# thangvubk/SoftGroup

Measured on AMD Instinct MI355X. Metric: scans/sec ScanNet-v2-like inference (softgroup_scannet.yaml, full forward_test), higher is better.
Workload: dtype f32

## Files before the change

### softgroup_amd/csrc/ballquery.hip

```cpp
#include "common.h"
#include "scan.h"

namespace sg {

constexpr int32_t kBqEmpty = 0x7f7f7f7f;
constexpr int kBqBuf = 2048;
constexpr int kBqCap = SG_BALLQUERY_MAX_NEIGHBORS;
constexpr int kBqKeep = 64;

struct BqWs {
  int4 *cell;
  int32_t *table;
  int32_t *count;
  int32_t *start;
  int32_t *cursor;
  int32_t *slot_of;
  float4 *sorted;
  int32_t *keep;
  void *scan_ws;
  size_t scan_bytes;
  uint32_t cap;
};

__device__ __forceinline__ uint32_t cell_slot(int b, int cx, int cy, int cz, uint32_t mask) {
  uint64_t h = (static_cast<uint64_t>(static_cast<uint32_t>(b)) << 32) | static_cast<uint32_t>(cx);
  h = mix64(h) ^ ((static_cast<uint64_t>(static_cast<uint32_t>(cy)) << 32) | static_cast<uint32_t>(cz));
  return static_cast<uint32_t>(mix64(h)) & mask;
}

__global__ void __launch_bounds__(256) bq_insert_kernel(const float *__restrict__ xyz,
                                                       const int32_t *__restrict__ batch_idxs,
                                                       int n, double inv_cell, int4 *__restrict__ cell,
                                                       int32_t *table, uint32_t mask, int32_t *count,
                                                       int32_t *__restrict__ slot_of) {
  const int i = blockIdx.x * 256 + threadIdx.x;
  if (i >= n) return;
  int4 c;
  c.x = batch_idxs ? batch_idxs[i] : 0;
  c.y = static_cast<int>(floor(static_cast<double>(xyz[3 * i + 0]) * inv_cell));
  c.z = static_cast<int>(floor(static_cast<double>(xyz[3 * i + 1]) * inv_cell));
  c.w = static_cast<int>(floor(static_cast<double>(xyz[3 * i + 2]) * inv_cell));
  cell[i] = c;
  uint32_t s = cell_slot(c.x, c.y, c.z, c.w, mask);
  while (true) {
    int32_t cur = __hip_atomic_load(&table[s], __ATOMIC_RELAXED, __HIP_MEMORY_SCOPE_AGENT);
    if (cur == kBqEmpty) {
      cur = atomicCAS(&table[s], kBqEmpty, i);
      if (cur == kBqEmpty) break;
    }
    int4 o;
    o.x = batch_idxs ? batch_idxs[cur] : 0;
    o.y = static_cast<int>(floor(static_cast<double>(xyz[3 * cur + 0]) * inv_cell));
    o.z = static_cast<int>(floor(static_cast<double>(xyz[3 * cur + 1]) * inv_cell));
    o.w = static_cast<int>(floor(static_cast<double>(xyz[3 * cur + 2]) * inv_cell));
    if (o.x == c.x && o.y == c.y && o.z == c.z && o.w == c.w) break;
    s = (s + 1) & mask;
  }
  slot_of[i] = static_cast<int32_t>(s);
  atomicAdd(&count[s], 1);
}

__global__ void __launch_bounds__(256) bq_scatter_kernel(const float *__restrict__ xyz, int n,
                                                        const int32_t *__restrict__ slot_of,
                                                        const int32_t *__restrict__ start,
                                                        int32_t *cursor, float4 *__restrict__ sorted) {
  const int i = blockIdx.x * 256 + threadIdx.x;
  if (i >= n) return;
  const int s = slot_of[i];
  const int pos = start[s] + atomicAdd(&cursor[s], 1);
  sorted[pos] = make_float4(xyz[3 * i], xyz[3 * i + 1], xyz[3 * i + 2], __int_as_float(i));
}

__device__ __forceinline__ float dist2(float ox, float oy, float oz, float x, float y, float z) {
  const float dx = __fsub_rn(ox, x), dy = __fsub_rn(oy, y), dz = __fsub_rn(oz, z);
  return __fmaf_rn(dz, dz, __fmaf_rn(dx, dx, __fmul_rn(dy, dy)));
}

struct BqCells {
  int start, excl, incl, total;
};
__device__ __forceinline__ BqCells bq_cells(int my_start, int my_count) {
  BqCells c;
  c.start = my_start;
  c.incl = wave_incl_scan(my_count);
  c.excl = c.incl - my_count;
  c.total = __shfl(c.incl, 63, 64);
  return c;
}
__device__ __forceinline__ int bq_candidate(const BqCells &c, int t) {
  int lo = 0, hi = 26;
#pragma unroll
  for (int it = 0; it < 5; ++it) {
    const int mid = (lo + hi) >> 1;
    const bool right = __shfl(c.incl, mid, 64) <= t;
    lo = right ? mid + 1 : lo;
    hi = right ? hi : mid;
  }
  return __shfl(c.start, lo, 64) + (t - __shfl(c.excl, lo, 64));
}

__device__ __forceinline__ int bq_scan_count(const float4 *__restrict__ sorted, const BqCells &c,
                                             float ox, float oy, float oz, float r2, int limit) {
  int total = 0;
  for (int t0 = 0; t0 < c.total; t0 += 64) {
    const int t = t0 + lane_id();
    const int at = bq_candidate(c, min(t, c.total - 1));
    if (t < c.total) {
      const float4 p = sorted[at];
      total += (dist2(ox, oy, oz, p.x, p.y, p.z) < r2 && __float_as_int(p.w) < limit) ? 1 : 0;
    }
  }
  return wave_sum(total);
}

template <bool FILL>
__global__ void __launch_bounds__(256) bq_query_kernel(const float *__restrict__ xyz, int n,
                                                      float r2, const int4 *__restrict__ cell,
                                                      const int32_t *__restrict__ table,
                                                      const int32_t *__restrict__ count,
                                                      const int32_t *__restrict__ start,
                                                      uint32_t mask, const float4 *__restrict__ sorted,
                                                      int32_t *__restrict__ start_len,
                                                      int32_t *__restrict__ idx_out, int32_t *__restrict__ keep) {
  __shared__ __attribute__((aligned(16))) int32_t buf_all[FILL ? 4 * kBqBuf : 4 * kBqKeep];
  const int wave = threadIdx.x >> 6, lane = threadIdx.x & 63;
  int32_t *buf = buf_all + wave * (FILL ? kBqBuf : kBqKeep);
  for (int i = blockIdx.x * 4 + wave; i < n; i += gridDim.x * 4) {
    if (FILL) {
      const int out_len = start_len[2 * i + 1];
      if (out_len <= kBqKeep) {
        if (lane < out_len) idx_out[static_cast<int64_t>(start_len[2 * i]) + lane] = keep[static_cast<int64_t>(i) * kBqKeep + lane];
        continue;
      }
    }
    const float ox = xyz[3 * i], oy = xyz[3 * i + 1], oz = xyz[3 * i + 2];
    const int4 c = cell[i];
    int my_start = 0, my_count = 0;
    if (lane < 27) {
      const int cx = c.y + lane / 9 - 1, cy = c.z + (lane / 3) % 3 - 1, cz = c.w + lane % 3 - 1;
      uint32_t s = cell_slot(c.x, cx, cy, cz, mask);
      while (true) {
        const int32_t rep = table[s];
        if (rep == kBqEmpty) break;
        const int4 o = cell[rep];
        if (o.x == c.x && o.y == cx && o.z == cy && o.w == cz) {
          my_start = start[s];
          my_count = count[s];
          break;
        }
        s = (s + 1) & mask;
      }
    }
    const BqCells cells = bq_cells(my_start, my_count);
    if (!FILL) {
      int m = 0;
      for (int t0 = 0; t0 < cells.total; t0 += 64) {
        const int t = t0 + lane;
        const int at = bq_candidate(cells, min(t, cells.total - 1));
        bool ok = false;
        int id = 0;
        if (t < cells.total) {
          const float4 p = sorted[at];
          id = __float_as_int(p.w);
          ok = dist2(ox, oy, oz, p.x, p.y, p.z) < r2;
        }
        const uint64_t bal = __ballot(ok);
        const int pos = m + mask_prefix(bal);
        if (ok && pos < kBqKeep) buf[pos] = id;
        m += __popcll(bal);
      }
      if (lane == 0) start_len[2 * i + 1] = min(m, kBqCap);
      if (m <= kBqKeep) {
        __builtin_amdgcn_fence(__ATOMIC_RELEASE, "wavefront");
        __builtin_amdgcn_wave_barrier();
        const int e = lane < m ? buf[lane] : 0x7fffffff;
        int rank = 0;
        for (int j = 0; j < m; ++j) rank += (buf[j] < e);
        if (lane < m) keep[static_cast<int64_t>(i) * kBqKeep + rank] = e;
      }
      __builtin_amdgcn_wave_barrier();
      continue;
    }
    const int out_start = start_len[2 * i], out_len = start_len[2 * i + 1];
    int limit = 0x7fffffff;
    int m = 0;
    for (int attempt = 0; attempt < 2; ++attempt) {
      m = 0;
      for (int t0 = 0; t0 < cells.total; t0 += 64) {
        const int t = t0 + lane;
        const int at = bq_candidate(cells, min(t, cells.total - 1));
        bool ok = false;
        int id = 0;
        if (t < cells.total) {
          const float4 p = sorted[at];
          id = __float_as_int(p.w);
          ok = dist2(ox, oy, oz, p.x, p.y, p.z) < r2 && id < limit;
        }
        const uint64_t bal = __ballot(ok);
        const int pos = m + mask_prefix(bal);
        if (ok && pos < kBqBuf) buf[pos] = id;
        m += __popcll(bal);
      }
      if (m <= kBqBuf) break;
      int lo = 0, hi = n;
      while (lo < hi) {
        const int mid = lo + (hi - lo) / 2;
        const int cmid = bq_scan_count(sorted, cells, ox, oy, oz, r2, mid);
        if (cmid >= out_len) hi = mid; else lo = mid + 1;
      }
      limit = lo;
    }
    __builtin_amdgcn_fence(__ATOMIC_RELEASE, "wavefront");
    __builtin_amdgcn_wave_barrier();
    for (int e0 = 0; e0 < m; e0 += 64) {
      const int ei = e0 + lane;
      const int e = ei < m ? buf[ei] : 0x7fffffff;
      int rank = 0;
      int j = 0;
      for (; j + 4 <= m; j += 4) {
        const int4 q = *reinterpret_cast<const int4 *>(buf + j);
        rank += (q.x < e) + (q.y < e) + (q.z < e) + (q.w < e);
      }
      for (; j < m; ++j) rank += (buf[j] < e);
      if (ei < m && rank < out_len) idx_out[static_cast<int64_t>(out_start) + rank] = e;
    }
    __builtin_amdgcn_wave_barrier();
  }
}

static size_t bq_cap(int n) {
  size_t cap = 1024;
  while (cap < static_cast<size_t>(n) * 2) cap <<= 1;
  return cap;
}

static bool bq_carve(void *ws, size_t ws_bytes, int n, BqWs *w) {
  Workspace a(ws, ws_bytes);
  const size_t nn = static_cast<size_t>(n > 0 ? n : 1);
  w->cap = static_cast<uint32_t>(bq_cap(n));
  w->cell = a.take<int4>(nn);
  w->sorted = a.take<float4>(nn);
  w->table = a.take<int32_t>(w->cap);
  w->count = a.take<int32_t>(w->cap);
  w->start = a.take<int32_t>(w->cap);
  w->cursor = a.take<int32_t>(w->cap);
  w->slot_of = a.take<int32_t>(nn);
  w->scan_bytes = scan_workspace_bytes(w->cap);
  w->scan_ws = a.take<char>(w->scan_bytes);
  w->keep = a.take<int32_t>(nn * kBqKeep);
  return w->scan_ws != nullptr && w->keep != nullptr;
}

}

using namespace sg;

extern "C" {

size_t sg_ballquery_workspace_bytes(int n) {
  const size_t nn = static_cast<size_t>(n > 0 ? n : 1);
  const size_t cap = bq_cap(n);
  return 2 * align_up(nn * 16) + 4 * align_up(cap * 4) + align_up(nn * 4) +
         align_up(scan_workspace_bytes(cap)) + align_up(nn * kBqKeep * 4) + 256;
}

int sg_ballquery_build_grid(const float *xyz, const int32_t *batch_idxs, int n, float radius,
                            void *ws, size_t ws_bytes, sg_stream_t stream_) {
  SG_REQUIRE(n >= 0 && radius > 0.f, "sg_ballquery_build_grid: bad arguments (n=%d r=%g)", n, radius);
  hipStream_t stream = as_stream(stream_);
  BqWs w;
  if (!bq_carve(ws, ws_bytes, n, &w)) {
    set_error("sg_ballquery_build_grid: workspace too small");
    return SG_ERR_WORKSPACE;
  }
  if (n == 0) return SG_OK;
  {
    FillList f;
    f.add(w.table, static_cast<size_t>(w.cap) * 4, 0x7f);
    f.add(w.count, static_cast<size_t>(w.cap) * 4, 0);
    f.add(w.cursor, static_cast<size_t>(w.cap) * 4, 0);
    fill_many(f, stream);
  }
  const double inv_cell = 1.0 / (static_cast<double>(radius) * (1.0 + 1e-6));
  const int grid = (n + 255) / 256;
  bq_insert_kernel<<<grid, 256, 0, stream>>>(xyz, batch_idxs, n, inv_cell, w.cell, w.table,
                                             w.cap - 1, w.count, w.slot_of);
  const int32_t *count = w.count;
  int32_t *start = w.start;
  auto in = [count] __device__(int64_t s) { return count[s]; };
  auto out = [start] __device__(int64_t s, int v) { start[s] = v; };
  int rc = exclusive_scan(in, out, w.cap, nullptr, w.scan_ws, w.scan_bytes, stream);
  if (rc != SG_OK) return rc;
  bq_scatter_kernel<<<grid, 256, 0, stream>>>(xyz, n, w.slot_of, w.start, w.cursor, w.sorted);
  return check_launch("sg_ballquery_build_grid");
}

int sg_ballquery_count(const float *xyz, const int32_t *batch_idxs, int n, float radius,
                       int32_t *start_len, int32_t *meta, void *ws, size_t ws_bytes,
                       sg_stream_t stream_) {
  (void)batch_idxs;
  (void)meta;
  SG_REQUIRE(n >= 0 && radius > 0.f, "sg_ballquery_count: bad arguments");
  BqWs w;
  if (!bq_carve(ws, ws_bytes, n, &w)) {
    set_error("sg_ballquery_count: workspace too small");
    return SG_ERR_WORKSPACE;
  }
  if (n == 0) return SG_OK;
  const float r2 = radius * radius;
  bq_query_kernel<false><<<grid_for(n, 4, 256 * 16), 256, 0, as_stream(stream_)>>>(
      xyz, n, r2, w.cell, w.table, w.count, w.start, w.cap - 1, w.sorted, start_len, nullptr, w.keep);
  return check_launch("sg_ballquery_count");
}

int sg_ballquery_fill(const float *xyz, const int32_t *batch_idxs, int n, float radius,
                      const int32_t *start_len, int32_t *idx, void *ws, size_t ws_bytes,
                      sg_stream_t stream_) {
  (void)batch_idxs;
  SG_REQUIRE(n >= 0 && radius > 0.f, "sg_ballquery_fill: bad arguments");
  BqWs w;
  if (!bq_carve(ws, ws_bytes, n, &w)) {
    set_error("sg_ballquery_fill: workspace too small");
    return SG_ERR_WORKSPACE;
  }
  if (n == 0) return SG_OK;
  const float r2 = radius * radius;
  bq_query_kernel<true><<<grid_for(n, 4, 256 * 16), 256, 0, as_stream(stream_)>>>(
      xyz, n, r2, w.cell, w.table, w.count, w.start, w.cap - 1, w.sorted,
      const_cast<int32_t *>(start_len), idx, w.keep);
  return check_launch("sg_ballquery_fill");
}

}
```

### softgroup_amd/csrc/bfs.hip

```cpp
#include <stdlib.h>

#include <map>
#include <mutex>
#include <utility>

#include "common.h"
#include "scan.h"

namespace sg {

constexpr int kCap = SG_BALLQUERY_MAX_NEIGHBORS;
constexpr int kEmitThreads = 512;
constexpr int kEmitWaves = kEmitThreads / 64;

#define SG_LD(p) __hip_atomic_load((p), __ATOMIC_RELAXED, __HIP_MEMORY_SCOPE_AGENT)
#define SG_ST(p, v) __hip_atomic_store((p), (v), __ATOMIC_RELAXED, __HIP_MEMORY_SCOPE_AGENT)

struct BfsWs {
  int32_t *parent, *lab, *size, *cid, *coff, *owner, *seeds, *ebase, *wcnt, *asym_nodes;
  int4 *label;
  int2 *erec;
  int32_t *counters;
  void *scan_ws;
  size_t scan_bytes;
// ... 1 lines not shown
  unsigned long long *big_rec[2];
};

constexpr int kBigFastWgs = 16;
constexpr int kBigSlice = 8192;
constexpr int kBigClusterMin = 16384;
inline bool big_fast_on() {
  const char *e = getenv("SG_BFS_BIG_FAST");
  return !(e && atoi(e) == 0);
}
inline int thin_levels_on() {
  const char *e = getenv("SG_BFS_THIN");
  return e ? atoi(e) : 0;
}
inline bool big_local_on() {
  const char *e = getenv("SG_BFS_BIG_LOCAL");
  return !(e && atoi(e) == 0);
}
inline size_t big_stage_entries(int n) {
  return n > kBigClusterMin && big_fast_on() ? static_cast<size_t>(n) + static_cast<size_t>(kBigFastWgs) * kBigSlice : 0;
}

static bool bfs_carve(void *ws, size_t ws_bytes, int n, int64_t n_edges, BfsWs *w) {
  Workspace a(ws, ws_bytes);
  const size_t nn = static_cast<size_t>(n > 0 ? n : 1);
  w->parent = a.take<int32_t>(nn);
  w->lab = a.take<int32_t>(nn);
  w->label = a.take<int4>(nn);
  w->size = a.take<int32_t>(nn);
  w->cid = a.take<int32_t>(nn);
  w->coff = a.take<int32_t>(nn);
  w->owner = a.take<int32_t>(nn);
  w->seeds = a.take<int32_t>(nn);
  w->ebase = a.take<int32_t>(nn);
  w->wcnt = a.take<int32_t>(nn);
  w->asym_nodes = a.take<int32_t>(nn);
  w->counters = a.take<int32_t>(64);
  w->scan_bytes = scan_workspace_bytes(n);
  w->scan_ws = a.take<char>(w->scan_bytes);
  w->erec = a.take<int2>(static_cast<size_t>(n_edges > 0 ? n_edges : 1));
  bool ok = w->scan_ws != nullptr && w->erec != nullptr;
  const size_t be = big_stage_entries(n);
  for (int i = 0; i < 2; ++i) {
    w->big_stage[i] = be ? a.take<int32_t>(be) : nullptr;
    w->big_rec[i] = be ? a.take<unsigned long long>(be) : nullptr;
    ok = ok && (be == 0 || (w->big_stage[i] != nullptr && w->big_rec[i] != nullptr));
  }
  return ok;
}

__device__ __forceinline__ int uf_find(int32_t *parent, int x) {
  int cur = SG_LD(&parent[x]);
  if (cur != x) {
    int prev = x, next;
    while (cur > (next = SG_LD(&parent[cur]))) {
      SG_ST(&parent[prev], next);
      prev = cur;
      cur = next;
    }
  }
  return cur;
}

__device__ __forceinline__ void uf_union(int32_t *parent, int a, int b) {
  while (a != b) {
    if (a < b) { const int t = a; a = b; b = t; }
    const int old = atomicCAS(&parent[a], a, b);
    if (old == a) return;
    a = uf_find(parent, old);
    b = uf_find(parent, b);
  }
}

__device__ __forceinline__ bool list_has_sorted(const int32_t *__restrict__ lst, int len, int key) {
  int lo = 0, hi = len;
  while (lo < hi) {
    const int mid = (lo + hi) >> 1;
    const int v = lst[mid];
    if (v < key) lo = mid + 1; else hi = mid;
  }
  return lo < len && lst[lo] == key;
}

__global__ void __launch_bounds__(256) bfs_init_kernel(int n, int32_t *parent, int32_t *size,
                                                      int32_t *owner) {
  const int i = blockIdx.x * 256 + threadIdx.x;
  if (i < n) {
    parent[i] = i;
    size[i] = 0;
    owner[i] = 0x7fffffff;
  }
}

constexpr int kSample = 2;
template <int SAMPLE>
__global__ void __launch_bounds__(256) bfs_union_kernel(const int32_t *__restrict__ idx,
                                                       const int32_t *__restrict__ start_len, int n,
                                                       int lists_sorted, int radius_lists,
                                                       int32_t *parent, int32_t *asym_nodes,
                                                       int32_t *counters) {
  const int wave = threadIdx.x >> 6, lane = threadIdx.x & 63;
  for (int u = blockIdx.x * 4 + wave; u < n; u += gridDim.x * 4) {
    const int st = start_len[2 * u], ln_all = start_len[2 * u + 1];
    const int ln = SAMPLE ? min(ln_all, kSample) : ln_all;
    const bool u_capped = ln_all >= kCap;
    bool any_asym = false;
    const int ru = SAMPLE ? -1 : SG_LD(&parent[u]);
    for (int p0 = 0; p0 < ln; p0 += 64) {
      const int p = p0 + lane;
      const int v = p < ln ? idx[st + p] : u;
      bool sym = true;
      if (v != u) {
        const int vst = start_len[2 * v], vln = start_len[2 * v + 1];
        if (!radius_lists || u_capped || vln >= kCap) {
          if (lists_sorted) {
            sym = list_has_sorted(idx + vst, vln, u);
          } else {
            sym = false;
            for (int j = 0; j < vln; ++j)
              if (idx[vst + j] == u) { sym = true; break; }
          }
        }
        if (sym) {
          if (v < u && (SAMPLE || SG_LD(&parent[v]) != ru)) uf_union(parent, uf_find(parent, u), uf_find(parent, v));
        }
      }
      any_asym |= !sym;
    }
    if (!SAMPLE && __any(any_asym)) {
      if (lane == 0) asym_nodes[atomicAdd(&counters[0], 1)] = u;
    }
  }
}

__global__ void __launch_bounds__(256) bfs_hook_min_kernel(const int32_t *__restrict__ idx,
                                                          const int32_t *__restrict__ start_len, int n,
                                                          int lists_sorted, int radius_lists, int32_t *parent) {
  const int u = blockIdx.x * 256 + threadIdx.x;
  if (u >= n) return;
  const int st = start_len[2 * u], ln = start_len[2 * u + 1];
  if (ln == 0 || !lists_sorted) return;
  const int v = idx[st];
  if (v >= u) return;
  if (!radius_lists || ln >= kCap || start_len[2 * v + 1] >= kCap)
    if (!list_has_sorted(idx + start_len[2 * v], start_len[2 * v + 1], u)) return;
  parent[u] = v;
}
__global__ void __launch_bounds__(256) bfs_compress_kernel(int n, int32_t *parent) {
  const int i = blockIdx.x * 256 + threadIdx.x;
  if (i < n) SG_ST(&parent[i], uf_find(parent, i));
}

__global__ void __launch_bounds__(256) bfs_flatten_kernel(int n, int32_t *parent, int32_t *lab) {
  const int i = blockIdx.x * 256 + threadIdx.x;
  if (i >= n) return;
  int r = i;
  while (true) {
    const int p = SG_LD(&parent[r]);
    if (p == r) break;
    r = p;
  }
  lab[i] = r;
}
__global__ void __launch_bounds__(256) bfs_store_root_kernel(int n, const int32_t *__restrict__ lab,
                                                            int32_t *__restrict__ parent) {
  const int i = blockIdx.x * 256 + threadIdx.x;
  if (i < n) parent[i] = lab[i];
}

__global__ void __launch_bounds__(256) bfs_propagate_kernel(const int32_t *__restrict__ idx,
                                                           const int32_t *__restrict__ start_len,
                                                           const int32_t *__restrict__ asym_nodes,
                                                           int n_asym,
                                                           const int32_t *__restrict__ root_of,
                                                           int32_t *lab, int32_t *counters) {
  const int wave = threadIdx.x >> 6, lane = threadIdx.x & 63;
  for (int a = blockIdx.x * 4 + wave; a < n_asym; a += gridDim.x * 4) {
    const int u = asym_nodes[a];
    const int ru = root_of[u];
    const int st = start_len[2 * u], ln = start_len[2 * u + 1];
    for (int p = lane; p < ln; p += 64) {
      const int rv = root_of[idx[st + p]];
      if (rv == ru) continue;
      const int lu = SG_LD(&lab[ru]);
      if (lu < SG_LD(&lab[rv])) {
        if (atomicMin(&lab[rv], lu) > lu) SG_ST(&counters[1], 1);
      }
    }
  }
}

__global__ void __launch_bounds__(256) bfs_label_kernel(int n, const int32_t *__restrict__ root_of,
                                                       const int32_t *__restrict__ lab,
                                                       const int32_t *__restrict__ start_len,
                                                       int4 *__restrict__ node_rec, int32_t *size) {
  const int i = blockIdx.x * 256 + threadIdx.x;
  const bool valid = i < n;
  const int l = valid ? lab[root_of[i]] : -1;
  int slot = 0;
  uint64_t todo = __ballot(valid);
  const int lane = threadIdx.x & 63;
  while (todo) {
    const int leader = __ffsll(static_cast<long long>(todo)) - 1;
    const int ll = __shfl(l, leader, 64);
    const uint64_t same = __ballot(valid && l == ll) & todo;
    int base = 0;
    if (lane == leader) base = atomicAdd(&size[ll], __popcll(same));
    base = __shfl(base, leader, 64);
    if ((same >> lane) & 1ull) slot = base + __popcll(same & ((1ull << lane) - 1ull));
    todo &= ~same;
  }
  if (!valid) return;
  node_rec[i] = make_int4(l, slot, start_len[2 * i], start_len[2 * i + 1]);
}

__global__ void __launch_bounds__(256) bfs_zero_size_kernel(int n, int32_t *size) {
  const int i = blockIdx.x * 256 + threadIdx.x;
  if (i < n) size[i] = 0;
}

__global__ void __launch_bounds__(256) bfs_owner_reset_kernel(int n, const int4 *__restrict__ label,
                                                             const int32_t *__restrict__ size,
                                                             int min_size, const int32_t *gate,
                                                             int32_t *__restrict__ owner) {
  if (SG_LD(gate) == 0) return;
  for (int i = blockIdx.x * 256 + threadIdx.x; i < n; i += gridDim.x * 256)
    if (size[label[i].x] > min_size) owner[i] = 0x7fffffff;
// ... 1321 lines not shown
    hipStreamDestroy(it->second.side);
    hipEventDestroy(it->second.fork);
    hipEventDestroy(it->second.join);
    hipEventDestroy(it->second.back);
  }
  g_bfs_side.erase(it);
}
struct BfsLabelNote {
  const void *ws = nullptr;
  int max_kept = -1;
};
static thread_local BfsLabelNote t_bfs_note;

void bfs_emit_defer(BfsDefer *d) { t_bfs_defer = d; }
int bfs_emit_join(const BfsDefer &d, hipStream_t stream) {
  if (!d.deferred) return SG_OK;
  BfsSide *side = bfs_side(stream);
  if (side == nullptr || side->side != d.side || hipEventRecord(side->join, side->side) != hipSuccess ||
      hipStreamWaitEvent(stream, side->join, 0) != hipSuccess) {
    set_error("bfs_emit_join: joining the side stream failed");
    return SG_ERR_LAUNCH;
  }
  return SG_OK;
}
int bfs_label_max_kept(const void *ws) { return t_bfs_note.ws == ws ? t_bfs_note.max_kept : -1; }

__global__ void __launch_bounds__(256) bfs_kept_members_kernel(const int32_t *__restrict__ l2p, int n_pts,
                                                              const int4 *__restrict__ label,
                                                              const int32_t *__restrict__ size,
                                                              const float *__restrict__ thr_dev,
                                                              int32_t *__restrict__ out) {
  __shared__ int wsum[4];
  const float thr = thr_dev[0];
  int mine = 0;
  for (int p = blockIdx.x * 256 + threadIdx.x; p < n_pts; p += gridDim.x * 256)
    mine += static_cast<float>(size[label[l2p[p]].x]) >= thr ? 1 : 0;
  const int w = wave_sum(mine);
  if ((threadIdx.x & 63) == 0) wsum[threadIdx.x >> 6] = w;
  __syncthreads();
  if (threadIdx.x == 0) atomicAdd(out, wsum[0] + wsum[1] + wsum[2] + wsum[3]);
}
int bfs_count_kept_members(const void *ws, size_t ws_bytes, int n, int64_t n_edges, const int32_t *l2p, int n_pts,
                           const float *thr_dev, int32_t *out, hipStream_t stream) {
  BfsWs w;
  if (!bfs_carve(const_cast<void *>(ws), ws_bytes, n, n_edges, &w)) {
    set_error("bfs_count_kept_members: workspace too small");
    return SG_ERR_WORKSPACE;
  }
  hipMemsetAsync(out, 0, 4, stream);
  bfs_kept_members_kernel<<<grid_for(n_pts, 256, 1024), 256, 0, stream>>>(l2p, n_pts, w.label, w.size, thr_dev, out);
  return check_launch("bfs_count_kept_members");
}

}

using namespace sg;

extern "C" {

size_t sg_bfs_workspace_bytes(int n, int64_t n_edges) {
  const size_t nn = static_cast<size_t>(n > 0 ? n : 1);
  const size_t ne = static_cast<size_t>(n_edges > 0 ? n_edges : 1);
  const size_t be = big_stage_entries(n);
  return 14 * align_up(nn * 4) + align_up(64 * 4) + align_up(scan_workspace_bytes(n)) +
         align_up(ne * sizeof(int2)) + 2 * (align_up(be * 4) + align_up(be * 8)) + 256;
}

int sg_bfs_cluster_label(const int32_t *bq_idxs, const int32_t *start_len, int n, int64_t n_edges,
                         int list_flags, const int32_t *seg_of_point, const float *seg_thr,
                         int n_seg, int32_t *n_cluster_host, int32_t *sum_npoint_host, void *ws,
                         size_t ws_bytes, sg_stream_t stream_) {
  SG_REQUIRE(n >= 0 && n_seg >= 1 && seg_thr != nullptr, "sg_bfs_cluster_label: bad arguments");
  hipStream_t stream = as_stream(stream_);
  BfsWs w;
  if (!bfs_carve(ws, ws_bytes, n, n_edges, &w)) {
    set_error("sg_bfs_cluster_label: workspace too small");
    return SG_ERR_WORKSPACE;
  }
  *n_cluster_host = 0;
  *sum_npoint_host = 0;
  if (n == 0) return SG_OK;
  const int grid = (n + 255) / 256;
  hipMemsetAsync(w.counters, 0, 64 * 4, stream);
  bfs_init_kernel<<<grid, 256, 0, stream>>>(n, w.parent, w.size, w.owner);
  static const bool one_pass = getenv("SG_BFS_ONE_PASS") != nullptr;
  if (!one_pass) {
    static const bool sample_env = getenv("SG_BFS_SAMPLE") != nullptr;
    if (sample_env || !(list_flags & SG_LISTS_SORTED))
      bfs_union_kernel<1><<<grid_for(n, 4, 256 * 16), 256, 0, stream>>>(bq_idxs, start_len, n,
                                                                      list_flags & SG_LISTS_SORTED,
                                                                      list_flags & SG_LISTS_RADIUS,
                                                                      w.parent, w.asym_nodes, w.counters);
    else
      bfs_hook_min_kernel<<<grid, 256, 0, stream>>>(bq_idxs, start_len, n, list_flags & SG_LISTS_SORTED,
                                                   list_flags & SG_LISTS_RADIUS, w.parent);
    bfs_compress_kernel<<<grid, 256, 0, stream>>>(n, w.parent);
  }
  bfs_union_kernel<0><<<grid_for(n, 4, 256 * 16), 256, 0, stream>>>(bq_idxs, start_len, n,
                                                                  list_flags & SG_LISTS_SORTED,
                                                                  list_flags & SG_LISTS_RADIUS,
                                                                  w.parent, w.asym_nodes, w.counters);
  bfs_flatten_kernel<<<grid, 256, 0, stream>>>(n, w.parent, w.lab);
  bfs_store_root_kernel<<<grid, 256, 0, stream>>>(n, w.lab, w.parent);

  int32_t *host_counters = pinned_words();
  SG_REQUIRE(host_counters != nullptr, "sg_bfs_cluster_label: pinned allocation failed");
  for (int i = 0; i < 5; ++i) host_counters[i] = 0;
  for (int pass = 0; pass < 2; ++pass) {
    if (pass == 1) {
      const int n_asym = host_counters[0];
      while (true) {
        hipMemsetAsync(w.counters + 1, 0, 4, stream);
        bfs_propagate_kernel<<<grid_for(n_asym, 4, 256 * 16), 256, 0, stream>>>(
            bq_idxs, start_len, w.asym_nodes, n_asym, w.parent, w.lab, w.counters);
        host_counters[8] = 0;
        hipMemcpyAsync(host_counters + 8, w.counters + 1, 4, hipMemcpyDeviceToHost, stream);
        if (hipStreamSynchronize(stream) != hipSuccess) return check_launch("bfs propagate");
        if (!host_counters[8]) break;
      }
      bfs_zero_size_kernel<<<grid, 256, 0, stream>>>(n, w.size);
    }
    bfs_label_kernel<<<grid, 256, 0, stream>>>(n, w.parent, w.lab, start_len, w.label, w.size);
    const int4 *label = w.label;
    const int32_t *size = w.size;
    int32_t *cid = w.cid, *coff = w.coff;
    auto keep = [label, size, seg_of_point, seg_thr] __device__(int64_t i) -> int {
      if (label[i].x != static_cast<int32_t>(i)) return 0;
      const float thr = seg_thr[seg_of_point ? seg_of_point[i] : 0];
      return static_cast<float>(size[i]) >= thr ? 1 : 0;
    };
    int32_t *max_kept = w.counters + 4;
    auto keep_size = [keep, size, max_kept] __device__(int64_t i) -> int {
      const int s = keep(i) ? size[i] : 0;
      if (s > kBigMin) atomicMax(max_kept, s);
      return s;
    };
    int rc = exclusive_scan(keep, [cid] __device__(int64_t i, int v) { cid[i] = v; }, n,
                            w.counters + 2, w.scan_ws, w.scan_bytes, stream);
    if (rc != SG_OK) return rc;
    rc = exclusive_scan(keep_size, [coff] __device__(int64_t i, int v) { coff[i] = v; }, n,
                        w.counters + 3, w.scan_ws, w.scan_bytes, stream);
    if (rc != SG_OK) return rc;
    hipMemcpyAsync(host_counters, w.counters, 5 * sizeof(int32_t), hipMemcpyDeviceToHost, stream);
    if (hipStreamSynchronize(stream) != hipSuccess) return check_launch("sg_bfs_cluster_label");
    if (host_counters[0] == 0) break;
    if (pass == 0) hipMemsetAsync(w.counters + 4, 0, 4, stream);
  }
  *n_cluster_host = host_counters[2];
  *sum_npoint_host = host_counters[3];
  t_bfs_note.ws = ws;
  t_bfs_note.max_kept = host_counters[4];
  return check_launch("sg_bfs_cluster_label");
}

int sg_bfs_cluster_emit(const int32_t *bq_idxs, const int32_t *start_len, int n, int64_t n_edges,
                        const int32_t *seg_of_point, const float *seg_thr, int n_cluster,
                        int sum_npoint, int32_t *cluster_idxs, int32_t *cluster_offsets, void *ws,
                        size_t ws_bytes, sg_stream_t stream_) {
  SG_REQUIRE(n >= 0 && n_cluster >= 0 && sum_npoint >= 0, "sg_bfs_cluster_emit: bad arguments");
  hipStream_t stream = as_stream(stream_);
  BfsWs w;
  if (!bfs_carve(ws, ws_bytes, n, n_edges, &w)) {
    set_error("sg_bfs_cluster_emit: workspace too small");
    return SG_ERR_WORKSPACE;
  }
  if (n_cluster == 0 || n == 0) {
    hipMemsetAsync(cluster_offsets, 0, 4, stream);
    return SG_OK;
  }
  bfs_seed_kernel<<<(n + 255) / 256, 256, 0, stream>>>(n, w.label, w.size, w.cid, w.coff,
                                                       seg_of_point, seg_thr, w.seeds,
                                                       cluster_offsets);
  bfs_edge_rec_kernel<<<grid_for(n, 4, 256 * 16), 256, 0, stream>>>(bq_idxs, w.label, w.cid, w.seeds, n,
                                                                     n_cluster, w.erec);
  static const bool want_stats = getenv("SG_BFS_STATS") != nullptr;
  int32_t *stats = nullptr;
  if (want_stats) {
    hipMalloc(&stats, 256 * 8 * 4);
// ... 135 lines not shown
```

### softgroup_amd/csrc/common.h

```cpp
#pragma once
#include <hip/hip_runtime.h>
#include <stdint.h>
#include <stdio.h>

#include "../../include/softgroup_hip.h"

namespace sg {

constexpr int kWave = 64;

void set_error(const char *fmt, ...);
int32_t *pinned_words();

inline hipStream_t as_stream(sg_stream_t s) { return reinterpret_cast<hipStream_t>(s); }

inline int check_launch(const char *what) {
  hipError_t e = hipGetLastError();
  if (e != hipSuccess) {
    set_error("%s: %s", what, hipGetErrorString(e));
    return SG_ERR_LAUNCH;
  }
  return SG_OK;
}

// ... 54 lines not shown
  v += dpp_or_zero<0x118>(v);
  v += dpp_or_zero<0x142, 0xa>(v);
  v += dpp_or_zero<0x143, 0xc>(v);
  return v;
}
__device__ __forceinline__ int wave_sum(int v) {
  return __builtin_amdgcn_readlane(wave_incl_scan(v), 63);
}
__device__ __forceinline__ int wave_max(int v) {
#pragma unroll
  for (int o = 32; o > 0; o >>= 1) v = max(v, __shfl_xor(v, o, 64));
  return v;
}

constexpr int kFillMax = 16;
struct FillList {
  uint32_t *p[kFillMax];
  size_t words[kFillMax];
  uint32_t pattern[kFillMax];
  int n = 0;
  void add(void *ptr, size_t bytes, int byte) {
    if (bytes == 0 || ptr == nullptr || n >= kFillMax) return;
    p[n] = static_cast<uint32_t *>(ptr);
    words[n] = bytes / 4;
    pattern[n] = 0x01010101u * static_cast<uint32_t>(byte & 0xff);
    ++n;
  }
};
static __global__ void __launch_bounds__(256) fill_many_kernel(FillList f) {
  const int r = blockIdx.y;
  uint32_t *p = f.p[r];
  const size_t w = f.words[r];
  const uint32_t v = f.pattern[r];
  const size_t head = (16 - (reinterpret_cast<uintptr_t>(p) & 15)) / 4 % 4;
  const size_t h = head < w ? head : w;
  const size_t quads = (w - h) / 4;
  uint4 *q = reinterpret_cast<uint4 *>(p + h);
  const uint4 vv = make_uint4(v, v, v, v);
  for (size_t i = blockIdx.x * 256ull + threadIdx.x; i < quads; i += gridDim.x * 256ull) q[i] = vv;
  if (blockIdx.x == 0) {
    if (threadIdx.x < h) p[threadIdx.x] = v;
    const size_t t0 = h + quads * 4;
    if (threadIdx.x < w - t0) p[t0 + threadIdx.x] = v;
  }
}
inline void fill_many(const FillList &f, hipStream_t stream) {
  if (f.n == 0) return;
  size_t mx = 0;
  for (int i = 0; i < f.n; ++i) mx = f.words[i] > mx ? f.words[i] : mx;
  const int gx = grid_for(static_cast<int64_t>(mx / 4 + 1), 256, 1024);
  fill_many_kernel<<<dim3(gx, f.n), 256, 0, stream>>>(f);
}

extern thread_local int t_conv_arith;
void conv_chain_begin(hipStream_t stream);
bool conv_chain_recording();
int conv_chain_end();
void conv_chain_abort();
int conv_chain_concat(const float *a, const float *b, int64_t rows, int ca, int cb, const float *scale,
                      const float *shift, float *out, float *out_act);
int conv_chain_bn_relu(const float *x, const float *scale, const float *shift, int64_t rows, int c, float *out);
int conv_chain_check_abort(const char *who);
int conv_gather_rows(const void *in, int num_in_rows, const int32_t *nbr, int M_out, int K, int Cin, int Cout,
                     const float *w_k8, const float *post_scale, const float *post_shift, const void *residual,
                     const float *act_scale, const float *act_shift, void *out_act, const int32_t *order,
                     const uint32_t *tile_mask, const int32_t *nbr_tiles, void *out, void *ws, size_t ws_bytes,
                     sg_stream_t stream, int in16, int out16, int res16);
int spconv_wgrad_layout(const void *in, int in_bf16, const void *g_out, int g_bf16, const int32_t *nbr_t, int M_out,
                        int K, int Cin, int Cout, float *dw, int out_oki, void *ws, size_t ws_bytes,
                        sg_stream_t stream);
struct PackJob {
  const float *w;
  float *out;
  int cout, kvol, cin, mode;
};
int spconv_pack_weights(const PackJob *jobs, int n, sg_stream_t stream);
size_t octree_stash_bytes(int n);
int octree_ballquery_count_stash(const float *points, const float *boxes, const int32_t *pt_inds,
                                 const int32_t *pt_start_len, int n, float radius, int32_t *start_len, int32_t *stash,
                                 hipStream_t stream);
int octree_ballquery_fill_stash(const float *points, const float *boxes, const int32_t *pt_inds,
                                const int32_t *pt_start_len, int n, float radius, const int32_t *start_len,
                                const int32_t *stash, int32_t *idx, hipStream_t stream);
void conv_release_stream(int dev, hipStream_t stream);
void unet_release_stream(int dev, hipStream_t stream);
void scan_release_stream(int dev, hipStream_t stream);
void bfs_release_stream(int dev, hipStream_t stream);
constexpr int kBfsGiantMin = 16384;
struct BfsDefer {
  bool deferred = false;
  hipStream_t side = nullptr;
};
void bfs_emit_defer(BfsDefer *d);
int bfs_emit_join(const BfsDefer &d, hipStream_t stream);
int bfs_label_max_kept(const void *ws);
int bfs_count_kept_members(const void *ws, size_t ws_bytes, int n, int64_t n_edges, const int32_t *l2p, int n_pts,
                           const float *thr_dev, int32_t *out, hipStream_t stream);

}
```

### softgroup_amd/csrc/scan_exec.hip

```cpp
#include <stdlib.h>
#include <string.h>

#include "common.h"
#include "scan.h"

namespace sg {

constexpr int kSelBlock = 256;
constexpr int kMaxSeg = 32;

__global__ void __launch_bounds__(kSelBlock) select_count_kernel(const float *__restrict__ scores, int n,
                                                                int n_cls, const int32_t *__restrict__ seg_class,
                                                                int n_seg, float thr, int n_blocks,
                                                                int32_t *__restrict__ blk_cnt) {
  __shared__ int part[4][kMaxSeg];
  const int i = blockIdx.x * kSelBlock + threadIdx.x;
  const int wave = threadIdx.x >> 6, lane = threadIdx.x & 63;
  for (int s = 0; s < n_seg; ++s) {
    const bool on = i < n && scores[static_cast<int64_t>(i) * n_cls + seg_class[s]] > thr;
    const int c = __popcll(__ballot(on));
    if (lane == 0) part[wave][s] = c;
  }
  __syncthreads();
  if (threadIdx.x < n_seg)
// ... 421 lines not shown
  const int C = cfg->feat_channels;
  SG_TAKE(cscale, float, n_prop);
  SG_TAKE(lo_s, float, 3 * static_cast<size_t>(n_prop));
  SG_TAKE(vox, int64_t, 4 * static_cast<size_t>(S));
  SG_TAKE(bad, int32_t, 64);
  hipMemsetAsync(bad, 0, sizeof(int32_t), stream);
  const float inv_ss = 1.0f / static_cast<float>(cfg->voxel_shape);
  proposal_box_kernel<<<n_prop < 1024 ? n_prop : 1024, 256, 0, stream>>>(pairs, poff, n_prop, coords_float, inv_ss,
                                                                        cfg->voxel_scale, cscale, lo_s);
  proposal_voxel_coords_kernel<<<grid_for(S, 256), 256, 0, stream>>>(pairs, S, coords_float, cscale, lo_s,
                                                                    cfg->voxel_shape, vox, bad);
  const size_t vx_bytes = sg_voxelize_idx_workspace_bytes(S);
  SG_TAKE(vx_ws, char, vx_bytes);
  SG_TAKE(inp_map, int32_t, S);
  SG_TRY(sg_voxelize_idx_build(vox, S, 4, 4, inp_map, meta + 40, vx_ws, vx_bytes, stream_));
  hipMemcpyAsync(meta + 42, bad, sizeof(int32_t), hipMemcpyDeviceToDevice, stream);
  SG_TRY(read_back(host, meta + 40, 3, stream, kWhat));
  const int M = host[0], mA = host[1];
  SG_REQUIRE(host[2] == 0, "%s: a proposal voxel coordinate fell outside [0, %d) "
             "(the reference asserts here, softgroup.py:698)", kWhat, cfg->voxel_shape);
  res->n_voxels = M;
  res->max_active = mA;
  SG_TAKE(vc64, int64_t, 4 * static_cast<size_t>(M));
  SG_TAKE(rules, int32_t, static_cast<size_t>(M) * (mA + 1));
  SG_TRY(sg_voxelize_idx_fill(vox, S, 4, 4, inp_map, M, mA, vc64, rules, vx_ws, vx_bytes, stream_));
  SG_TAKE(vc32, int32_t, 4 * static_cast<size_t>(M));
  SG_TAKE(vox_off, int32_t, static_cast<size_t>(n_prop) + 1);
  SG_TAKE(vfeat, float, static_cast<size_t>(M) * C);
  proposal_voxel_pack_kernel<<<grid_for(M, 256), 256, 0, stream>>>(vc64, M, n_prop, vc32, vox_off);
  proposal_voxel_feats_kernel<<<grid_for(static_cast<int64_t>(M) * C, 256), 256, 0, stream>>>(
      point_feats, pairs, rules, M, mA, C, vfeat);
  res->voxel_coords = ar.at(vc32);
  res->voxel_offsets = ar.at(vox_off);
  res->voxel_feats = ar.at(vfeat);
  res->point_to_voxel = ar.at(inp_map);
  res->arena_used = ar.off;
  return check_launch(kWhat);
}

extern "C" {

int sg_scan_grouping(const sg_grouping_cfg *cfg, const float *scores, const float *pt_offsets,
                     const float *coords_float, const int32_t *batch_idxs, const float *point_feats,
                     void *arena, size_t arena_bytes, sg_grouping_result *res, sg_stream_t stream_) {
  static const char *kWhat = "sg_scan_grouping";
  SG_REQUIRE(cfg != nullptr && res != nullptr, "sg_scan_grouping: null descriptor");
  SG_REQUIRE(cfg->n_points >= 0 && cfg->n_sem_classes >= 1 && cfg->n_seg >= 0 && cfg->n_seg <= kMaxSeg &&
                 cfg->batch_size >= 1 && cfg->feat_channels >= 1 && cfg->voxel_shape >= 0,
             "sg_scan_grouping: bad configuration (n_seg must be <= %d)", kMaxSeg);
  memset(res, 0, sizeof(*res));
  hipStream_t stream = as_stream(stream_);
  int32_t *host = pinned_words();
  SG_REQUIRE(host != nullptr, "sg_scan_grouping: no pinned host words");
  ScanArena ar(arena, arena_bytes);
  const int n = cfg->n_points, n_seg = cfg->n_seg;
  if (n == 0 || n_seg == 0) return SG_OK;

  const int n_blocks = (n + kSelBlock - 1) / kSelBlock;
  SG_TAKE(meta, int32_t, 64);
  SG_TAKE(blk_cnt, int32_t, static_cast<size_t>(n_seg) * n_blocks);
  SG_TAKE(blk_off, int32_t, static_cast<size_t>(n_seg) * n_blocks);
  select_count_kernel<<<n_blocks, kSelBlock, 0, stream>>>(scores, n, cfg->n_sem_classes, cfg->seg_class, n_seg,
                                                         cfg->score_thr, n_blocks, blk_cnt);
  select_scan_kernel<<<1, 1024, 0, stream>>>(blk_cnt, n_seg, n_blocks, cfg->min_npoint, blk_off, meta);
  SG_TRY(check_launch(kWhat));
  SG_TRY(read_back(host, meta, 1, stream, kWhat));
  const int n_sel = host[0];
  res->n_selected = n_sel;
  if (n_sel == 0) return SG_OK;
  SG_TAKE(obj, int32_t, n_sel);
  SG_TAKE(seg_of, int32_t, n_sel);
  SG_TAKE(pts, float, 3 * static_cast<size_t>(n_sel));
  SG_TAKE(key, int32_t, n_sel);
  select_emit_kernel<<<n_blocks, kSelBlock, 0, stream>>>(scores, n, cfg->n_sem_classes, cfg->seg_class, n_seg,
                                                        cfg->score_thr, n_blocks, blk_off, coords_float,
                                                        pt_offsets, batch_idxs, cfg->batch_size, obj, seg_of,
                                                        pts, key);

  const size_t bq_bytes = sg_ballquery_workspace_bytes(n_sel);
  SG_TAKE(bq_ws, char, bq_bytes);
  SG_TAKE(start_len, int32_t, 2 * static_cast<size_t>(n_sel));
  const size_t sc_bytes = sg_scan_workspace_bytes(n_sel);
  SG_TAKE(sc_ws, char, sc_bytes);
  hipMemsetAsync(start_len, 0, sizeof(int32_t) * 2 * n_sel, stream);
  SG_TRY(sg_ballquery_build_grid(pts, key, n_sel, cfg->radius, bq_ws, bq_bytes, stream_));
  SG_TRY(sg_ballquery_count(pts, key, n_sel, cfg->radius, start_len, nullptr, bq_ws, bq_bytes, stream_));
  SG_TRY(sg_exclusive_scan_startlen(start_len, n_sel, meta + 32, sc_ws, sc_bytes, stream_));
  SG_TRY(read_back(host, meta + 32, 1, stream, kWhat));
  const int n_active = host[0];
  res->n_neighbours = n_active;
  SG_TAKE(bq_idx, int32_t, n_active);
  SG_TRY(sg_ballquery_fill(pts, key, n_sel, cfg->radius, start_len, bq_idx, bq_ws, bq_bytes, stream_));

  const size_t bfs_bytes = sg_bfs_workspace_bytes(n_sel, n_active);
  SG_TAKE(bfs_ws, char, bfs_bytes);
  int32_t n_prop = 0, S = 0;
  SG_TRY(sg_bfs_cluster_label(bq_idx, start_len, n_sel, n_active, SG_LISTS_SORTED | SG_LISTS_RADIUS, seg_of,
                              cfg->seg_thr, n_seg, &n_prop, &S, bfs_ws, bfs_bytes, stream_));
  res->n_proposals = n_prop;
  res->sum_npoint = S;
  if (S == 0) return SG_OK;
  SG_TAKE(pairs, int32_t, 2 * static_cast<size_t>(S));
  SG_TAKE(poff, int32_t, static_cast<size_t>(n_prop) + 1);
  hipMemsetAsync(poff, 0, sizeof(int32_t) * (n_prop + 1), stream);
  if (t_scan_emit_hook != nullptr) t_scan_emit_hook(t_scan_emit_ctx);
  SG_TRY(sg_bfs_cluster_emit(bq_idx, start_len, n_sel, n_active, seg_of, cfg->seg_thr, n_prop, S, pairs, poff,
                             bfs_ws, bfs_bytes, stream_));
  proposal_map_kernel<<<grid_for(S, 256), 256, 0, stream>>>(pairs, S, obj);
  res->proposals_idx = ar.at(pairs);
  res->proposals_offset = ar.at(poff);
  if (cfg->voxel_shape == 0) {
    res->arena_used = ar.off;
    return check_launch(kWhat);
  }

  return voxelise_proposals(cfg, pairs, poff, n_prop, S, coords_float, point_feats, ar, meta, host, res, stream_, kWhat);
}

int sg_scan_grouping_pp(const sg_grouping_pp_cfg *pcfg, const float *scores, const float *pt_offsets,
                        const float *coords_float, const int32_t *batch_idxs, const float *point_feats,
                        void *arena, size_t arena_bytes, sg_grouping_result *res, sg_stream_t stream_) {
  static const char *kWhat = "sg_scan_grouping_pp";
  SG_REQUIRE(pcfg != nullptr && res != nullptr, "sg_scan_grouping_pp: null descriptor");
  const sg_grouping_cfg *cfg = &pcfg->base;
  SG_REQUIRE(cfg->n_points >= 0 && cfg->n_sem_classes >= 1 && cfg->n_seg >= 0 && cfg->n_seg <= kMaxSeg &&
                 cfg->batch_size >= 1 && cfg->feat_channels >= 1 && cfg->voxel_shape >= 0,
             "sg_scan_grouping_pp: bad configuration (n_seg must be <= %d)", kMaxSeg);
  SG_REQUIRE(pcfg->radius > 0 && (!pcfg->with_pyramid || pcfg->base_size > 0),
             "sg_scan_grouping_pp: radius and pyramid_base_size must be positive");
  memset(res, 0, sizeof(*res));
  hipStream_t stream = as_stream(stream_);
  int32_t *host = pinned_words();
  SG_REQUIRE(host != nullptr, "sg_scan_grouping_pp: no pinned host words");
  ScanArena ar(arena, arena_bytes);
  const int n = cfg->n_points, n_seg = cfg->n_seg;
  if (n == 0 || n_seg == 0) return SG_OK;

  const int n_blocks = (n + kSelBlock - 1) / kSelBlock;
  SG_TAKE(meta, int32_t, 128);
  SG_TAKE(blk_cnt, int32_t, static_cast<size_t>(n_seg) * n_blocks);
  SG_TAKE(blk_off, int32_t, static_cast<size_t>(n_seg) * n_blocks);
  select_count_kernel<<<n_blocks, kSelBlock, 0, stream>>>(scores, n, cfg->n_sem_classes, cfg->seg_class, n_seg,
                                                         cfg->score_thr, n_blocks, blk_cnt);
  select_scan_kernel<<<1, 1024, 0, stream>>>(blk_cnt, n_seg, n_blocks, cfg->min_npoint, blk_off, meta);
  SG_TRY(check_launch(kWhat));
  SG_TRY(read_back(host, meta, 1 + n_seg, stream, kWhat));
  const int n_sel = host[0];
  int count[kMaxSeg];
  for (int s = 0; s < n_seg; ++s) count[s] = host[1 + s];
  res->n_selected = n_sel;
  if (n_sel == 0) return SG_OK;
  SG_TAKE(obj, int32_t, n_sel);
  SG_TAKE(seg_of, int32_t, n_sel);
  SG_TAKE(pts, float, 3 * static_cast<size_t>(n_sel));
  SG_TAKE(key, int32_t, n_sel);
  select_emit_kernel<<<n_blocks, kSelBlock, 0, stream>>>(scores, n, cfg->n_sem_classes, cfg->seg_class, n_seg,
                                                        cfg->score_thr, n_blocks, blk_off, coords_float,
                                                        pt_offsets, batch_idxs, cfg->batch_size, obj, seg_of,
                                                        pts, key);
  SG_TAKE(pairs, int32_t, 2 * static_cast<size_t>(n_sel));
  SG_TAKE(poff, int32_t, static_cast<size_t>(n_sel) + 2);
  int n_prop = 0, S = 0;
  int64_t n_nbr = 0;
  const size_t loop_mark0 = ar.off;
  size_t loop_mark = loop_mark0;
  bool hook_pending = t_scan_emit_hook != nullptr;
  const bool defer_on = !(getenv("SG_PP_DEFER") && atoi(getenv("SG_PP_DEFER")) == 0);
  BfsDefer def;
// ... 247 lines not shown
```

Before: 415.7.

## Precompute per-cell neighbor ranges and skip list-symmetry checks when no lists capped

Ball query now builds a per-occupied-cell table of 27 neighbor cell ranges once, so count and fill kernels index it through a representative instead of re-probing the hash table per point. BFS init flags whether any neighbor list hit the cap. When none did, union and hook kernels take a cheaper path that relies on radius-list symmetry and exits early on sorted lists. The start_len memset is folded into the grid-build batched fill. This adds an extra kernel and extra workspace, and the shortcut correctness depends on symmetric uncapped lists.

New measurement: 407.5. -2.0%, worse.

```diff
diff --git a/softgroup_amd/csrc/ballquery.hip b/softgroup_amd/csrc/ballquery.hip
--- a/softgroup_amd/csrc/ballquery.hip
+++ b/softgroup_amd/csrc/ballquery.hip
@@ -15,6 +15,10 @@
   int32_t *start;
   int32_t *cursor;
   int32_t *slot_of;
+  int32_t *rep_of;
+  int2 *nbr;
+  int32_t *cell_list;
+  int32_t *n_cells;
   float4 *sorted;
   int32_t *keep;
   void *scan_ws;
@@ -32,7 +36,9 @@
                                                        const int32_t *__restrict__ batch_idxs,
                                                        int n, double inv_cell, int4 *__restrict__ cell,
                                                        int32_t *table, uint32_t mask, int32_t *count,
-                                                       int32_t *__restrict__ slot_of) {
+                                                       int32_t *__restrict__ slot_of,
+                                                       int32_t *__restrict__ rep_of,
+                                                       int32_t *__restrict__ cell_list, int32_t *n_cells) {
   const int i = blockIdx.x * 256 + threadIdx.x;
   if (i >= n) return;
   int4 c;
@@ -42,12 +48,17 @@
   c.w = static_cast<int>(floor(static_cast<double>(xyz[3 * i + 2]) * inv_cell));
   cell[i] = c;
   uint32_t s = cell_slot(c.x, c.y, c.z, c.w, mask);
+  int32_t rep = i;
   while (true) {
     int32_t cur = __hip_atomic_load(&table[s], __ATOMIC_RELAXED, __HIP_MEMORY_SCOPE_AGENT);
     if (cur == kBqEmpty) {
       cur = atomicCAS(&table[s], kBqEmpty, i);
-      if (cur == kBqEmpty) break;
-    }
+      if (cur == kBqEmpty) {
+        cell_list[atomicAdd(n_cells, 1)] = i;
+        break;
+      }
+    }
+    rep = cur;
     int4 o;
     o.x = batch_idxs ? batch_idxs[cur] : 0;
     o.y = static_cast<int>(floor(static_cast<double>(xyz[3 * cur + 0]) * inv_cell));
@@ -55,8 +66,10 @@
     o.w = static_cast<int>(floor(static_cast<double>(xyz[3 * cur + 2]) * inv_cell));
     if (o.x == c.x && o.y == c.y && o.z == c.z && o.w == c.w) break;
     s = (s + 1) & mask;
+    rep = i;
   }
   slot_of[i] = static_cast<int32_t>(s);
+  rep_of[i] = rep;
   atomicAdd(&count[s], 1);
 }
 
@@ -69,6 +82,36 @@
   const int s = slot_of[i];
   const int pos = start[s] + atomicAdd(&cursor[s], 1);
   sorted[pos] = make_float4(xyz[3 * i], xyz[3 * i + 1], xyz[3 * i + 2], __int_as_float(i));
+}
+
+__global__ void __launch_bounds__(256) bq_cells_kernel(const int32_t *__restrict__ n_cells,
+                                                      const int32_t *__restrict__ cell_list,
+                                                      const int4 *__restrict__ cell,
+                                                      const int32_t *__restrict__ table,
+                                                      const int32_t *__restrict__ count,
+                                                      const int32_t *__restrict__ start, uint32_t mask,
+                                                      int2 *__restrict__ nbr) {
+  const int nc = n_cells[0];
+  const int sub = threadIdx.x & 31;
+  if (sub >= 27) return;
+  for (int g = blockIdx.x * 8 + (threadIdx.x >> 5); g < nc; g += gridDim.x * 8) {
+    const int rep = cell_list[g];
+    const int4 c = cell[rep];
+    const int cx = c.y + sub / 9 - 1, cy = c.z + (sub / 3) % 3 - 1, cz = c.w + sub % 3 - 1;
+    int2 range = make_int2(0, 0);
+    uint32_t s = cell_slot(c.x, cx, cy, cz, mask);
+    while (true) {
+      const int32_t other = table[s];
+      if (other == kBqEmpty) break;
+      const int4 o = cell[other];
+      if (o.x == c.x && o.y == cx && o.z == cy && o.w == cz) {
+        range = make_int2(start[s], count[s]);
+        break;
+      }
+      s = (s + 1) & mask;
+    }
+    nbr[static_cast<int64_t>(rep) * 27 + sub] = range;
+  }
 }
 
 __device__ __forceinline__ float dist2(float ox, float oy, float oz, float x, float y, float z) {
@@ -115,11 +158,9 @@
 
 template <bool FILL>
 __global__ void __launch_bounds__(256) bq_query_kernel(const float *__restrict__ xyz, int n,
-                                                      float r2, const int4 *__restrict__ cell,
-                                                      const int32_t *__restrict__ table,
-                                                      const int32_t *__restrict__ count,
-                                                      const int32_t *__restrict__ start,
-                                                      uint32_t mask, const float4 *__restrict__ sorted,
+                                                      float r2, const int32_t *__restrict__ rep_of,
+                                                      const int2 *__restrict__ nbr,
+                                                      const float4 *__restrict__ sorted,
                                                       int32_t *__restrict__ start_len,
                                                       int32_t *__restrict__ idx_out, int32_t *__restrict__ keep) {
   __shared__ __attribute__((aligned(16))) int32_t buf_all[FILL ? 4 * kBqBuf : 4 * kBqKeep];
@@ -134,22 +175,11 @@
       }
     }
     const float ox = xyz[3 * i], oy = xyz[3 * i + 1], oz = xyz[3 * i + 2];
-    const int4 c = cell[i];
     int my_start = 0, my_count = 0;
     if (lane < 27) {
-      const int cx = c.y + lane / 9 - 1, cy = c.z + (lane / 3) % 3 - 1, cz = c.w + lane % 3 - 1;
-      uint32_t s = cell_slot(c.x, cx, cy, cz, mask);
-      while (true) {
-        const int32_t rep = table[s];
-        if (rep == kBqEmpty) break;
-        const int4 o = cell[rep];
-        if (o.x == c.x && o.y == cx && o.z == cy && o.w == cz) {
-          my_start = start[s];
-          my_count = count[s];
-          break;
-        }
-        s = (s + 1) & mask;
-      }
+      const int2 range = nbr[static_cast<int64_t>(rep_of[i]) * 27 + lane];
+      my_start = range.x;
+      my_count = range.y;
     }
     const BqCells cells = bq_cells(my_start, my_count);
     if (!FILL) {
@@ -245,29 +275,19 @@
   w->start = a.take<int32_t>(w->cap);
   w->cursor = a.take<int32_t>(w->cap);
   w->slot_of = a.take<int32_t>(nn);
+  w->rep_of = a.take<int32_t>(nn);
   w->scan_bytes = scan_workspace_bytes(w->cap);
   w->scan_ws = a.take<char>(w->scan_bytes);
   w->keep = a.take<int32_t>(nn * kBqKeep);
-  return w->scan_ws != nullptr && w->keep != nullptr;
-}
-
-}
-
-using namespace sg;
-
-extern "C" {
-
-size_t sg_ballquery_workspace_bytes(int n) {
-  const size_t nn = static_cast<size_t>(n > 0 ? n : 1);
-  const size_t cap = bq_cap(n);
-  return 2 * align_up(nn * 16) + 4 * align_up(cap * 4) + align_up(nn * 4) +
-         align_up(scan_workspace_bytes(cap)) + align_up(nn * kBqKeep * 4) + 256;
-}
-
-int sg_ballquery_build_grid(const float *xyz, const int32_t *batch_idxs, int n, float radius,
-                            void *ws, size_t ws_bytes, sg_stream_t stream_) {
+  w->nbr = a.take<int2>(nn * 27);
+  w->cell_list = a.take<int32_t>(nn);
+  w->n_cells = a.take<int32_t>(1);
+  return w->scan_ws != nullptr && w->keep != nullptr && w->nbr != nullptr && w->n_cells != nullptr;
+}
+
+int ballquery_build_grid_clear(const float *xyz, const int32_t *batch_idxs, int n, float radius, void *ws,
+                               size_t ws_bytes, void *clear, size_t clear_bytes, hipStream_t stream) {
   SG_REQUIRE(n >= 0 && radius > 0.f, "sg_ballquery_build_grid: bad arguments (n=%d r=%g)", n, radius);
-  hipStream_t stream = as_stream(stream_);
   BqWs w;
   if (!bq_carve(ws, ws_bytes, n, &w)) {
     set_error("sg_ballquery_build_grid: workspace too small");
@@ -279,12 +299,14 @@
     f.add(w.table, static_cast<size_t>(w.cap) * 4, 0x7f);
     f.add(w.count, static_cast<size_t>(w.cap) * 4, 0);
     f.add(w.cursor, static_cast<size_t>(w.cap) * 4, 0);
+    f.add(w.n_cells, 4, 0);
+    f.add(clear, clear_bytes, 0);
     fill_many(f, stream);
   }
   const double inv_cell = 1.0 / (static_cast<double>(radius) * (1.0 + 1e-6));
   const int grid = (n + 255) / 256;
   bq_insert_kernel<<<grid, 256, 0, stream>>>(xyz, batch_idxs, n, inv_cell, w.cell, w.table,
-                                             w.cap - 1, w.count, w.slot_of);
+                                             w.cap - 1, w.count, w.slot_of, w.rep_of, w.cell_list, w.n_cells);
   const int32_t *count = w.count;
   int32_t *start = w.start;
   auto in = [count] __device__(int64_t s) { return count[s]; };
@@ -292,7 +314,27 @@
   int rc = exclusive_scan(in, out, w.cap, nullptr, w.scan_ws, w.scan_bytes, stream);
   if (rc != SG_OK) return rc;
   bq_scatter_kernel<<<grid, 256, 0, stream>>>(xyz, n, w.slot_of, w.start, w.cursor, w.sorted);
+  bq_cells_kernel<<<grid_for(static_cast<int64_t>(n) * 32, 256, 2048), 256, 0, stream>>>(
+      w.n_cells, w.cell_list, w.cell, w.table, w.count, w.start, w.cap - 1, w.nbr);
   return check_launch("sg_ballquery_build_grid");
+}
+
+}
+
+using namespace sg;
+
+extern "C" {
+
+size_t sg_ballquery_workspace_bytes(int n) {
+  const size_t nn = static_cast<size_t>(n > 0 ? n : 1);
+  const size_t cap = bq_cap(n);
+  return 2 * align_up(nn * 16) + 4 * align_up(cap * 4) + 3 * align_up(nn * 4) +
+         align_up(scan_workspace_bytes(cap)) + align_up(nn * kBqKeep * 4) + align_up(nn * 27 * 8) + 2 * 256;
+}
+
+int sg_ballquery_build_grid(const float *xyz, const int32_t *batch_idxs, int n, float radius,
+                            void *ws, size_t ws_bytes, sg_stream_t stream_) {
+  return ballquery_build_grid_clear(xyz, batch_idxs, n, radius, ws, ws_bytes, nullptr, 0, as_stream(stream_));
 }
 
 int sg_ballquery_count(const float *xyz, const int32_t *batch_idxs, int n, float radius,
@@ -309,7 +351,7 @@
   if (n == 0) return SG_OK;
   const float r2 = radius * radius;
   bq_query_kernel<false><<<grid_for(n, 4, 256 * 16), 256, 0, as_stream(stream_)>>>(
-      xyz, n, r2, w.cell, w.table, w.count, w.start, w.cap - 1, w.sorted, start_len, nullptr, w.keep);
+      xyz, n, r2, w.rep_of, w.nbr, w.sorted, start_len, nullptr, w.keep);
   return check_launch("sg_ballquery_count");
 }
 
@@ -326,7 +368,7 @@
   if (n == 0) return SG_OK;
   const float r2 = radius * radius;
   bq_query_kernel<true><<<grid_for(n, 4, 256 * 16), 256, 0, as_stream(stream_)>>>(
-      xyz, n, r2, w.cell, w.table, w.count, w.start, w.cap - 1, w.sorted,
+      xyz, n, r2, w.rep_of, w.nbr, w.sorted,
       const_cast<int32_t *>(start_len), idx, w.keep);
   return check_launch("sg_ballquery_fill");
 }
diff --git a/softgroup_amd/csrc/bfs.hip b/softgroup_amd/csrc/bfs.hip
--- a/softgroup_amd/csrc/bfs.hip
+++ b/softgroup_amd/csrc/bfs.hip
@@ -107,14 +107,19 @@
   return lo < len && lst[lo] == key;
 }
 
-__global__ void __launch_bounds__(256) bfs_init_kernel(int n, int32_t *parent, int32_t *size,
-                                                      int32_t *owner) {
+constexpr int kAnyCapped = 5;
+__global__ void __launch_bounds__(256) bfs_init_kernel(int n, const int32_t *__restrict__ start_len,
+                                                      int32_t *parent, int32_t *size, int32_t *owner,
+                                                      int32_t *counters) {
   const int i = blockIdx.x * 256 + threadIdx.x;
+  bool capped = false;
   if (i < n) {
     parent[i] = i;
     size[i] = 0;
     owner[i] = 0x7fffffff;
-  }
+    capped = start_len[2 * i + 1] >= kCap;
+  }
+  if (__any(capped) && (threadIdx.x & 63) == 0) atomicOr(&counters[kAnyCapped], 1);
 }
 
 constexpr int kSample = 2;
@@ -125,6 +130,19 @@
                                                        int32_t *parent, int32_t *asym_nodes,
                                                        int32_t *counters) {
   const int wave = threadIdx.x >> 6, lane = threadIdx.x & 63;
+  if (!SAMPLE && lists_sorted && radius_lists && counters[kAnyCapped] == 0) {
+    for (int u = blockIdx.x * 4 + wave; u < n; u += gridDim.x * 4) {
+      const int st = start_len[2 * u], ln = start_len[2 * u + 1];
+      const int ru = SG_LD(&parent[u]);
+      for (int p0 = 0; p0 < ln; p0 += 64) {
+        const int p = p0 + lane;
+        const int v = p < ln ? idx[st + p] : u;
+        if (v < u && SG_LD(&parent[v]) != ru) uf_union(parent, uf_find(parent, u), uf_find(parent, v));
+        if (__any(v >= u)) break;
+      }
+    }
+    return;
+  }
   for (int u = blockIdx.x * 4 + wave; u < n; u += gridDim.x * 4) {
     const int st = start_len[2 * u], ln_all = start_len[2 * u + 1];
     const int ln = SAMPLE ? min(ln_all, kSample) : ln_all;
@@ -160,14 +178,15 @@
 
 __global__ void __launch_bounds__(256) bfs_hook_min_kernel(const int32_t *__restrict__ idx,
                                                           const int32_t *__restrict__ start_len, int n,
-                                                          int lists_sorted, int radius_lists, int32_t *parent) {
+                                                          int lists_sorted, int radius_lists, int32_t *parent,
+                                                          const int32_t *__restrict__ counters) {
   const int u = blockIdx.x * 256 + threadIdx.x;
   if (u >= n) return;
   const int st = start_len[2 * u], ln = start_len[2 * u + 1];
   if (ln == 0 || !lists_sorted) return;
   const int v = idx[st];
   if (v >= u) return;
-  if (!radius_lists || ln >= kCap || start_len[2 * v + 1] >= kCap)
+  if (!radius_lists || (counters[kAnyCapped] != 0 && (ln >= kCap || start_len[2 * v + 1] >= kCap)))
     if (!list_has_sorted(idx + start_len[2 * v], start_len[2 * v + 1], u)) return;
   parent[u] = v;
 }
@@ -1655,7 +1674,7 @@
   if (n == 0) return SG_OK;
   const int grid = (n + 255) / 256;
   hipMemsetAsync(w.counters, 0, 64 * 4, stream);
-  bfs_init_kernel<<<grid, 256, 0, stream>>>(n, w.parent, w.size, w.owner);
+  bfs_init_kernel<<<grid, 256, 0, stream>>>(n, start_len, w.parent, w.size, w.owner, w.counters);
   static const bool one_pass = getenv("SG_BFS_ONE_PASS") != nullptr;
   if (!one_pass) {
     static const bool sample_env = getenv("SG_BFS_SAMPLE") != nullptr;
@@ -1666,7 +1685,7 @@
                                                                       w.parent, w.asym_nodes, w.counters);
     else
       bfs_hook_min_kernel<<<grid, 256, 0, stream>>>(bq_idxs, start_len, n, list_flags & SG_LISTS_SORTED,
-                                                   list_flags & SG_LISTS_RADIUS, w.parent);
+                                                   list_flags & SG_LISTS_RADIUS, w.parent, w.counters);
     bfs_compress_kernel<<<grid, 256, 0, stream>>>(n, w.parent);
   }
   bfs_union_kernel<0><<<grid_for(n, 4, 256 * 16), 256, 0, stream>>>(bq_idxs, start_len, n,
diff --git a/softgroup_amd/csrc/common.h b/softgroup_amd/csrc/common.h
--- a/softgroup_amd/csrc/common.h
+++ b/softgroup_amd/csrc/common.h
@@ -160,6 +160,8 @@
 int octree_ballquery_fill_stash(const float *points, const float *boxes, const int32_t *pt_inds,
                                 const int32_t *pt_start_len, int n, float radius, const int32_t *start_len,
                                 const int32_t *stash, int32_t *idx, hipStream_t stream);
+int ballquery_build_grid_clear(const float *xyz, const int32_t *batch_idxs, int n, float radius, void *ws,
+                               size_t ws_bytes, void *clear, size_t clear_bytes, hipStream_t stream);
 void conv_release_stream(int dev, hipStream_t stream);
 void unet_release_stream(int dev, hipStream_t stream);
 void scan_release_stream(int dev, hipStream_t stream);
diff --git a/softgroup_amd/csrc/scan_exec.hip b/softgroup_amd/csrc/scan_exec.hip
--- a/softgroup_amd/csrc/scan_exec.hip
+++ b/softgroup_amd/csrc/scan_exec.hip
@@ -527,8 +527,8 @@
   SG_TAKE(start_len, int32_t, 2 * static_cast<size_t>(n_sel));
   const size_t sc_bytes = sg_scan_workspace_bytes(n_sel);
   SG_TAKE(sc_ws, char, sc_bytes);
-  hipMemsetAsync(start_len, 0, sizeof(int32_t) * 2 * n_sel, stream);
-  SG_TRY(sg_ballquery_build_grid(pts, key, n_sel, cfg->radius, bq_ws, bq_bytes, stream_));
+  SG_TRY(ballquery_build_grid_clear(pts, key, n_sel, cfg->radius, bq_ws, bq_bytes, start_len,
+                                    sizeof(int32_t) * 2 * n_sel, stream));
   SG_TRY(sg_ballquery_count(pts, key, n_sel, cfg->radius, start_len, nullptr, bq_ws, bq_bytes, stream_));
   SG_TRY(sg_exclusive_scan_startlen(start_len, n_sel, meta + 32, sc_ws, sc_bytes, stream_));
   SG_TRY(read_back(host, meta + 32, 1, stream, kWhat));
```
